# quarterwave0/LithographySimulator

Hardware: AMD Instinct MI355X
Metric: Abbe source-points x image-pixels per second (higher is better)
Workload: dtype f32

## Files before the change

lithographysimulator_amd/csrc/engine_kernels.hpp:

```cpp
#pragma once
#include <hip/hip_runtime.h>

#include "engine_common.hpp"
#include "abbe_plan.hpp"
#include "fft_core.hpp"
#include "wave_fft.hpp"

namespace litho {

template <int LOG2N>
struct Launch {
    using F = LineFFT<LOG2N, +1>;
    static constexpr int L = (F::T >= 64) ? 1 : 64 / F::T;
    static constexpr int THREADS = F::T * L;
#ifndef LITHO_NBUF
#define LITHO_NBUF 1
#endif
    static constexpr int NBUF = (LOG2N <= 12) ? LITHO_NBUF : 1;
    static constexpr size_t LDS_EXCH = (size_t)L * NBUF * F::LDS_LINE;
    static constexpr size_t LDS_BYTES = sizeof(float2) * (LDS_EXCH + F::LDS_TW);
#ifndef LITHO_WG_PER_CU
#define LITHO_WG_PER_CU 3
#endif
    static constexpr int WG_PER_CU = LOG2N <= 12 ? LITHO_WG_PER_CU : (LOG2N == 13 ? 2 : 1);
    static constexpr int WAVES = (THREADS / 256 > 0 ? THREADS / 256 : 1) * WG_PER_CU;
};


typedef unsigned int u32x2 __attribute__((ext_vector_type(2)));
static constexpr unsigned BUF_OOB = 0xFFFF0000u;

__device__ __forceinline__ __amdgpu_buffer_rsrc_t make_rsrc(const void* base, size_t bytes) {
    return __builtin_amdgcn_make_buffer_rsrc(const_cast<void*>(base), 0, (int)(unsigned)bytes, 0x00020000);
}
__device__ __forceinline__ float2 buf_load_c64(__amdgpu_buffer_rsrc_t r, unsigned off) {
    const u32x2 v = __builtin_amdgcn_raw_buffer_load_b64(r, off, 0, 0);
    return make_float2(__uint_as_float(v.x), __uint_as_float(v.y));
}
#ifndef LITHO_XSTORE_AUX
#define LITHO_XSTORE_AUX 16
#endif
template <int LOG2N> inline constexpr int t_store_aux = LOG2N >= 11 ? LITHO_XSTORE_AUX : 0;
typedef unsigned int u32x4 __attribute__((ext_vector_type(4)));
template <int AUX = 0>
__device__ __forceinline__ void buf_store_c64x2(__amdgpu_buffer_rsrc_t r, unsigned off, float2 a, float2 b) {
    u32x4 w;
    w.x = __float_as_uint(a.x); w.y = __float_as_uint(a.y);
    w.z = __float_as_uint(b.x); w.w = __float_as_uint(b.y);
    __builtin_amdgcn_raw_buffer_store_b128(w, r, off, 0, AUX);
}
template <int AUX = 0>
__device__ __forceinline__ void buf_store_c64(__amdgpu_buffer_rsrc_t r, unsigned off, float2 v) {
    u32x2 w;
    w.x = __float_as_uint(v.x);
    w.y = __float_as_uint(v.y);
    __builtin_amdgcn_raw_buffer_store_b64(w, r, off, 0, AUX);
}

__device__ __forceinline__ unsigned t_offset(const PassGeom& g, unsigned a, unsigned q) {
    return ((((q >> g.tcl) * g.rows + a) << g.tcl) + (q & ((1u << g.tcl) - 1u)));
}

typedef unsigned int uint2v __attribute__((ext_vector_type(2)));

__device__ __forceinline__ void touch_vgpr(float2& v) { asm volatile("" : "+v"(v.x), "+v"(v.y)); }
__device__ __forceinline__ void diag_keep(float2 v, unsigned o) { asm volatile("" ::"v"(v.x), "v"(v.y), "v"(o)); }

__device__ __forceinline__ const float* pack_weights() { return nullptr; }
__device__ __forceinline__ const float* pack_weights(const float* w) { return w; }

template <int LOG2N, int RL, bool PRUNED, int NP, int RP = 1, typename... Wt>
__global__ __launch_bounds__(Launch<LOG2N>::THREADS, (RP == 2 ? Launch<LOG2N>::WAVES / Launch<LOG2N>::WG_PER_CU * 2 : Launch<LOG2N>::WAVES)) void k_xpass_abbe(
    const float2* __restrict__ P, const float2* __restrict__ M, const int* __restrict__ shifts,
    float2* __restrict__ Tbuf, const float2* __restrict__ twtab, PassGeom g, int nb, int chunk, Wt... wts)
{
    constexpr bool WT = sizeof...(Wt) != 0;
    static_assert(sizeof...(Wt) <= 1 && !(WT && RP == 2), "weighted x-pass: one weight list, one row per workgroup (a weighted call ignores the row-pair knob)");
    [[maybe_unused]] const float* weights = pack_weights(wts...);
    using F = LineFFT<LOG2N, +1>;
    using LC = Launch<LOG2N>;
    constexpr unsigned IN = PRUNED ? natural_in_mask(RL) : 0xFFFFu;
    constexpr unsigned OUT = out_mask(RL);
    extern __shared__ __attribute__((aligned(16))) unsigned char smem_raw[];
    float2* smem = reinterpret_cast<float2*>(smem_raw);
    const int lt = threadIdx.x % F::T, lg = threadIdx.x / F::T;
    float2* lds = smem + (size_t)lg * LC::NBUF * F::LDS_LINE;

    typename F::Twiddles tw;
    F::load_twiddles(tw, twtab, lt, smem + LC::LDS_EXCH, threadIdx.x, LC::THREADS);

    static_assert(RP == 1 || (RP == 2 && NP == 1 && LC::L == 1), "row pairs: one plane, one line per workgroup");
    int a;
    if constexpr (LC::L == 1) {
        const int b = blockIdx.x, xcd = b & 7, i = b >> 3;
        a = ((i >> 2) * 32 + xcd * 4 + (i & 3)) * RP;
    } else {
        a = blockIdx.x * LC::L + lg;
    }
    const bool active = a < g.rows;
    const bool active1 = a + 1 < g.rows;
    const int r = g.ky0 + g.c + a;
    const size_t plane_bytes = (size_t)g.pn * g.pn * sizeof(float2);
    const __amdgpu_buffer_rsrc_t rM = make_rsrc(M, plane_bytes);

    unsigned koff[16];
    float2 pv[NP * RP][16];
    static_for<0, 16>([&](auto e_) {
        constexpr int e = decltype(e_)::value;
        if constexpr ((IN >> e) & 1u) {
            int k;
            const bool ok = centred_index(lt + F::T * e, F::N, g.kx0, g.kx1, k) && active;
            koff[e] = ok ? (unsigned)(g.c + k) : BUF_OOB;
        }
    });
    static_for<0, NP * RP>([&](auto p_) {
        constexpr int p = decltype(p_)::value;
        const __amdgpu_buffer_rsrc_t rP = make_rsrc(P + (size_t)(RP == 1 ? p : 0) * g.pn * g.pn, plane_bytes);
        static_for<0, 16>([&](auto e_) {
            constexpr int e = decltype(e_)::value;
            if constexpr ((IN >> e) & 1u)
                pv[p][e] = buf_load_c64(rP, koff[e] != BUF_OOB ? ((unsigned)(r + (RP == 1 ? 0 : p)) * g.pn + koff[e]) * 8u : BUF_OOB);
        });
    });
    unsigned toff[16];
    static_for<0, 16>([&](auto m_) {
        constexpr int m = decltype(m_)::value;
        if constexpr ((OUT >> m) & 1u) {
            int u;
            const bool ok = centred_index(lt + F::T * m, F::N, -g.c, g.pn - g.c, u) && active;
            const unsigned q = (unsigned)(u + g.c);
            toff[m] = ok ? t_offset(g, a, q) * 8u : BUF_OOB;
        }
    });

    const int s_begin = blockIdx.y * chunk;
    const int s_end = min(nb, s_begin + chunk);
    auto load_window = [&](int s, int rr, float2 (&mv)[16]) {
        const int dy = shifts[2 * s], dx = shifts[2 * s + 1];
        const unsigned mrow = (unsigned)(r + rr + dy) * g.pn + dx;
        static_for<0, 16>([&](auto e_) {
            constexpr int e = decltype(e_)::value;
            if constexpr ((IN >> e) & 1u)
#ifdef LITHO_DIAG_XNOLOAD
                mv[e] = make_float2((float)((mrow + koff[e]) & 1023u), 1.0f);
#else
                mv[e] = buf_load_c64(rM, koff[e] != BUF_OOB ? (mrow + koff[e]) * 8u : BUF_OOB);
#endif
        });
    };

    int flip = 0;
    float2 mnext[16];
    [[maybe_unused]] float wnext = 1.f;
    if (s_begin < s_end) load_window(s_begin, 0, mnext);
    if constexpr (WT) { if (s_begin < s_end) wnext = weights[s_begin]; }
    static_for<0, 16>([&](auto e_) {
        constexpr int e = decltype(e_)::value;
        if constexpr ((IN >> e) & 1u) touch_vgpr(mnext[e]);
    });
    const unsigned row1 = active1 ? (8u << g.tcl) : 0x80000000u;
    float2 held[RP == 2 ? 16 : 1];
    const bool hi8 = (threadIdx.x & 8) != 0;
    unsigned offc = 0, offd = 0;
    if constexpr (RP == 2) {
        const unsigned tileb = (unsigned)g.rows * (8u << g.tcl);
        offc = hi8 ? row1 - tileb : 0u;
        offd = hi8 ? 0u : row1 + tileb;
    }
    for (int s = s_begin; s < s_end; ++s) {
        static_for<0, RP>([&](auto rr_) {
            constexpr int rr = decltype(rr_)::value;
            float2 mv[16];
            static_for<0, 16>([&](auto e_) {
                constexpr int e = decltype(e_)::value;
                if constexpr ((IN >> e) & 1u) mv[e] = mnext[e];
            });
            [[maybe_unused]] float amp = 1.f;
            if constexpr (WT) amp = sqrtf(wnext);
#ifndef LITHO_XPASS_NO_PREFETCH
            if constexpr (rr + 1 < RP) load_window(s, rr + 1, mnext);
            else load_window(s + 1 < s_end ? s + 1 : s, 0, mnext);
#else
            if constexpr (rr + 1 < RP) load_window(s, rr + 1, mnext);
            else if (s + 1 < s_end) load_window(s + 1, 0, mnext);
#endif
            if constexpr (WT) {
                wnext = weights[s + 1 < s_end ? s + 1 : s];
                static_for<0, 16>([&](auto e_) {
                    constexpr int e = decltype(e_)::value;
                    if constexpr ((IN >> e) & 1u) mv[e] = make_float2(amp * mv[e].x, amp * mv[e].y);
                });
            }
            static_for<0, NP>([&](auto p_) {
                constexpr int p = decltype(p_)::value;
                float2 x[16];
                static_for<0, 16>([&](auto e_) {
                    constexpr int e = decltype(e_)::value;
                    if constexpr ((IN >> e) & 1u) x[e] = cmul(pv[RP == 1 ? p : rr][e], mv[e]);
                    else x[e] = make_float2(0.f, 0.f);
                });
                F::template run<LC::NBUF>(x, tw, lds, lt, flip);
                const __amdgpu_buffer_rsrc_t rT =
                    make_rsrc(Tbuf + ((size_t)p * nb + s) * g.t_point, (size_t)g.t_point * sizeof(float2));
                if constexpr (RP == 2 && rr == 0) {
                    static_for<0, 16>([&](auto m_) { held[decltype(m_)::value] = x[decltype(m_)::value]; });
                } else {
                    static_for<0, 16>([&](auto m_) {
                        constexpr int m = decltype(m_)::value;
#ifdef LITHO_DIAG_XNOSTORE
                        if constexpr ((OUT >> m) & 1u) diag_keep(x[m], toff[m]);
#elif defined(LITHO_DIAG_XSTORE_L2)
                        if constexpr ((OUT >> m) & 1u) buf_store_c64(rT, toff[m] == BUF_OOB ? BUF_OOB : (toff[m] & 0xFFFFFu), x[m]);
#else
                        if constexpr ((OUT >> m) & 1u) {
                            if constexpr (RP == 2) {
                                if (active) {
                                    const float bx = __uint_as_float(__builtin_amdgcn_update_dpp(0u, __float_as_uint(x[m].x), 0x128, 0xF, 0xF, false));
                                    const float by = __uint_as_float(__builtin_amdgcn_update_dpp(0u, __float_as_uint(x[m].y), 0x128, 0xF, 0xF, false));
                                    buf_store_c64<t_store_aux<LOG2N>>(rT, toff[m] + offc, hi8 ? make_float2(bx, by) : held[m]);
                                    buf_store_c64<t_store_aux<LOG2N>>(rT, toff[m] + offd, hi8 ? held[m] : make_float2(bx, by));
                                }
                            } else {
                                buf_store_c64<t_store_aux<LOG2N>>(rT, toff[m], x[m]);
                            }
                        }
#endif
                    });
                }
            });
        });
    }
}

template <int LOG2N, typename... Wt>
__global__ __launch_bounds__(Launch<LOG2N - 1>::THREADS, Launch<LOG2N - 1>::WAVES) void k_xpass_split(
    const float2* __restrict__ P, const float2* __restrict__ M, const int* __restrict__ shifts,
    float2* __restrict__ Tbuf, const float2* __restrict__ twtab, PassGeom g, int nb, int chunk, Wt... wts)
{
    constexpr bool WT = sizeof...(Wt) != 0;
    static_assert(sizeof...(Wt) <= 1, "one weight list");
    [[maybe_unused]] const float* weights = pack_weights(wts...);
    using F = LineFFT<LOG2N - 1, +1>;
    using LC = Launch<LOG2N - 1>;
    static_assert(LC::L == 1, "split x-pass: one row per workgroup");
    constexpr unsigned IN = natural_in_mask(0), OUT = out_mask(1);
    extern __shared__ __attribute__((aligned(16))) unsigned char smem_raw[];
    float2* smem = reinterpret_cast<float2*>(smem_raw);
    const int lt = threadIdx.x;
    float2* lds = smem;

    typename F::Twiddles tw;
// ... 680 lines not shown
```

lithographysimulator_amd/csrc/wave_kernels.hpp:

```cpp
#pragma once
#include "engine_kernels.hpp"

namespace litho {

template <int LOG2N>
struct WaveShape {
    static_assert(LOG2N >= 10 && LOG2N <= 12, "wave-per-line y-pass: N = 1024 .. 4096 (N = 8192: k_ypass_pair)");
    static constexpr int LS = LOG2N / 2;
    static constexpr int D = 1 << (LOG2N - 2 * LS);
    using W = WaveSq<LS>;
    static constexpr int S = W::S;
    static constexpr int THREADS = 256;
    static constexpr int UNITS = THREADS / S;
    static constexpr int COLS = UNITS / D;
    static constexpr int TILES = COLS / 4;
    static constexpr int JLIVE = S * D / 8;
    static constexpr size_t LDS_BYTES = (size_t)(THREADS / 64) * W::LDS_FLOATS * sizeof(float);
#ifndef LITHO_WAVE32_MINWAVES
#define LITHO_WAVE32_MINWAVES 4
#endif
    static constexpr int MINWAVES = LS == 5 ? LITHO_WAVE32_MINWAVES : 2;
};

template <int TC, int COLS>
__device__ __forceinline__ int wave_first_column(int b)
{
    constexpr int WPT = TC > COLS ? TC / COLS : 1;
    if constexpr (WPT == 1) return b * COLS;
    else return (((b / (8 * WPT)) * 8 + (b & 7)) * TC) + ((b >> 3) % WPT) * COLS;
}
template <int TC, int COLS>
static inline int wave_grid_x(int pn)
{
    constexpr int WPT = TC > COLS ? TC / COLS : 1;
    if constexpr (WPT == 1) return (pn + COLS - 1) / COLS;
    else return WPT * (((pn + TC - 1) / TC + 7) / 8 * 8);
}

typedef unsigned int u32x4v __attribute__((ext_vector_type(4)));
#ifndef LITHO_YLOAD_AUX
#define LITHO_YLOAD_AUX 0
#endif

template <int LOG2N, int TC, bool FULL = false>
__global__ __launch_bounds__(WaveShape<LOG2N>::THREADS, WaveShape<LOG2N>::MINWAVES) void k_ypass_wave(
    const float2* __restrict__ Tbuf, float* __restrict__ slab, const float2* __restrict__ twtab,
    PassGeom g, int nb, int G, int gstride)
{
    static_assert(TC == 4 || TC == 8, "T tiles are 4 or 8 columns wide");
    using WS = WaveShape<LOG2N>;
    using W = typename WS::W;
    static_assert(!FULL || WS::D == 1, "full-output variant: one unit per column");
    constexpr int S = WS::S, D = WS::D, JLIVE = FULL ? 2 * WS::JLIVE : WS::JLIVE, N = 1 << LOG2N;
    constexpr int NACC = FULL ? S : S / 2;
    auto kept_k2 = [](int i) constexpr { return FULL ? i : (i < S / 4 ? i : S / 2 + i); };
    extern __shared__ __attribute__((aligned(16))) unsigned char smem_raw[];
    float* smem = reinterpret_cast<float*>(smem_raw);
    const int lane = threadIdx.x & 63, wv = threadIdx.x >> 6;
    const int l = lane & (S - 1);
    const int unit = wv * W::LINES + (lane >> WS::LS);
    const int p = unit % D;
    const int colg = unit / D;
    float* lds = smem + wv * W::LDS_FLOATS;
    typename W::LaneTwiddles tw;
    float2* twlds = reinterpret_cast<float2*>(smem_raw + WS::LDS_BYTES);
    if constexpr (FULL) {
        W::fill_lane_twiddle_table(twlds, twtab, D, threadIdx.x, WS::THREADS);
        __syncthreads();
    } else {
        W::load_lane_twiddles(tw, twtab, l, D);
    }
    const float2 tl = twtab[l * p];

    const int qx = wave_first_column<TC, WS::COLS>(blockIdx.x) + colg;
    const int tile = __builtin_amdgcn_readfirstlane(qx / TC);
    const int col = qx & (TC - 1);
    const int plane = blockIdx.y / G, grp = blockIdx.y - plane * G;
    Tbuf += (size_t)plane * nb * g.t_point;
    slab += (size_t)plane * gstride * g.nt * 4 * g.pn;
    const bool active = tile * TC < g.pn;
    float acc[NACC];
    static_for<0, NACC>([&](auto i) { acc[i] = 0.f; });

    constexpr int RB = 8 * TC;
    const unsigned tile_bytes = active ? (unsigned)g.rows * RB : 0u;
    const unsigned vb = (unsigned)(l - g.ky0) * RB + (unsigned)col * 8u;
    auto slot_off = [&](int j) { return vb + (unsigned)(j <= JLIVE ? RB * S * j : RB * S * j - RB * S * S); };

    for (int s = grp; s < nb; s += G) {
#ifndef LITHO_WAVE_FULL_NOSYNC
        if constexpr (FULL) __builtin_amdgcn_s_barrier();
#endif
        const __amdgpu_buffer_rsrc_t rT =
            make_rsrc(Tbuf + (size_t)s * g.t_point + (size_t)(active ? tile : 0) * g.rows * TC, tile_bytes);
        float2 x[S];
#ifndef LITHO_WAVE_FULL_NOPAIR
        if constexpr (FULL && TC == 8) {
            float2* const mine = reinterpret_cast<float2*>(lds);
            float2* const theirs = reinterpret_cast<float2*>(smem + (wv ^ 1) * W::LDS_FLOATS);
            const unsigned vbp = vb - (unsigned)(col & 1) * 8u;
            auto pair_off = [&](int j) { return vbp + (unsigned)(j <= JLIVE ? RB * S * j : RB * S * j - RB * S * S); };
            static_for<JLIVE + 1, S - JLIVE>([&](auto j_) { x[decltype(j_)::value] = make_float2(0.f, 0.f); });
            const bool even_wave = (__builtin_amdgcn_readfirstlane(wv) & 1) == 0;
            if (even_wave) {
                static_for<0, JLIVE + 1>([&](auto j_) {
                    constexpr int j = decltype(j_)::value;
                    const u32x4v v = __builtin_amdgcn_raw_buffer_load_b128(rT, pair_off(j), 0, 0);
                    x[j] = make_float2(__uint_as_float(v.x), __uint_as_float(v.y));
                    theirs[j * 64 + lane] = make_float2(__uint_as_float(v.z), __uint_as_float(v.w));
                });
            } else {
                static_for<S - JLIVE, S>([&](auto j_) {
                    constexpr int j = decltype(j_)::value;
                    const u32x4v v = __builtin_amdgcn_raw_buffer_load_b128(rT, pair_off(j), 0, 0);
                    x[j] = make_float2(__uint_as_float(v.z), __uint_as_float(v.w));
                    theirs[(j - (S - JLIVE)) * 64 + lane] = make_float2(__uint_as_float(v.x), __uint_as_float(v.y));
                });
            }
            __syncthreads();
            if (even_wave) {
                static_for<S - JLIVE, S>([&](auto j_) { constexpr int j = decltype(j_)::value; x[j] = mine[(j - (S - JLIVE)) * 64 + lane]; });
            } else {
                static_for<0, JLIVE + 1>([&](auto j_) { constexpr int j = decltype(j_)::value; x[j] = mine[j * 64 + lane]; });
            }
            asm volatile("" ::: "memory");
        } else
#endif
        static_for<0, S>([&](auto j_) {
            constexpr int j = decltype(j_)::value;
            if constexpr (j <= JLIVE || j >= S - JLIVE) {
                float2 v = buf_load_c64(rT, slot_off(j));
                if constexpr (D > 1) {
                    if (p) {
                        constexpr int e = (S * j) % N;
                        constexpr double ang = 6.283185307179586476925 * e / N;
                        constexpr float sgn = (j >= S - JLIVE) ? -1.f : 1.f;
                        const float2 cj = make_float2(sgn * (float)__builtin_cos(ang), sgn * (float)__builtin_sin(ang));
                        v = cmul(cmul(v, cj), tl);
                    }
                }
                x[j] = v;
            } else {
                x[j] = make_float2(0.f, 0.f);
            }
        });
        if constexpr (FULL) W::template run_lds_tw<true>(x, twlds, lds, lane);
        else W::run(x, tw, lds, lane);
        static_for<0, NACC>([&](auto i_) {
            constexpr int i = decltype(i_)::value;
            constexpr int k2 = kept_k2(i);
            const float2 v = x[W::brev(k2)];
            acc[i] = fmaf(v.x, v.x, fmaf(v.y, v.y, acc[i]));
        });
    }

    if (!active || qx >= g.pn) return;
    float* srow = slab + ((size_t)grp * g.nt * 4 + qx) * g.pn;
    static_for<0, NACC>([&](auto i_) {
        constexpr int i = decltype(i_)::value;
        constexpr int k2 = kept_k2(i);
        const int n = l + S * k2;
        const int v = n < S * S / 2 ? n : n - S * S;
        srow[D * v + p + g.c] += acc[i];
    });
}

template <int NW>
struct CoopShape {
    static_assert(NW == 4, "four waves share four columns (32 bytes) of a tile row");
    static constexpr int S = 64, N = 4096, JLIVE = 16, NLIVE = 2 * JLIVE + 1;
    static constexpr int STAGE_FLOATS = NLIVE * 64 * 2 + 16;
    static constexpr int WAVE_FLOATS = STAGE_FLOATS >= WaveSq<6>::LDS_FLOATS ? STAGE_FLOATS : WaveSq<6>::LDS_FLOATS + 16;
    static_assert(WAVE_FLOATS >= WaveSq<6>::LDS_FLOATS, "the staging area holds the transpose matrix");
    static constexpr size_t LDS_BYTES = NW * (size_t)WAVE_FLOATS * sizeof(float) + (size_t)WaveSq<6>::TW_LDS_FLOAT2 * sizeof(float2);
    static constexpr int PARTS = 16 / NW;
    static inline int grid_x(int pn) { return PARTS * (((pn + 15) / 16 + 7) / 8 * 8); }
};

#ifdef LITHO_DIAG_COOP_NOLOAD
#define COOP_LOAD(r, off) u32x4v{(off), 0x3f800000u, (off) >> 3, 0x3f000000u}
#else
#define COOP_LOAD(r, off) __builtin_amdgcn_raw_buffer_load_b128(r, off, 0, 0)
#endif
template <int LOG2N, int NW>
__global__ __launch_bounds__(64 * NW, 2) void k_ypass_coop(
    const float2* __restrict__ Tbuf, float* __restrict__ slab, const float2* __restrict__ twtab,
    PassGeom g, int nb, int G, int gstride)
{
    static_assert(LOG2N == 12, "cooperative-loading y-pass over 16-column tiles: N = 4096");
    using W = WaveSq<6>;
    using CS = CoopShape<NW>;
    constexpr int S = CS::S, N = CS::N, JLIVE = CS::JLIVE, NLIVE = CS::NLIVE, TC = 16, RB = 8 * TC;
    constexpr int PART_BYTES = 8 * NW;
    extern __shared__ __attribute__((aligned(16))) unsigned char smem_raw[];
    float* smem = reinterpret_cast<float*>(smem_raw);
// ... 225 lines not shown
            prefetch(snext);
        }
        W::dft_dif(x);
#endif
        static_for<0, S>([&](auto i_) {
            constexpr int i = decltype(i_)::value;
            const float2 v = x[W::brev(i)];
            acc[i] = fmaf(v.x, v.x, fmaf(v.y, v.y, acc[i]));
        });
    }
    if (!active || qx >= g.pn) return;
    float* srow = slab + ((size_t)grp * g.nt * 4 + qx) * g.pn;
    static_for<0, S>([&](auto i_) {
        constexpr int i = decltype(i_)::value;
        const int n = lane + S * i;
        const int v = n < S * S / 2 ? n : n - S * S;
        srow[v + g.c] += acc[i];
    });
}

template <int LOG2N, int TC>
__global__ __launch_bounds__(256, 2) void k_ypass_pair(
    const float2* __restrict__ Tbuf, float* __restrict__ slab, const float2* __restrict__ twtab,
    PassGeom g, int nb, int G, int gstride)
{
    static_assert(LOG2N == 13, "pair-of-waves y-pass: N = 8192");
    using W = WaveSq<6>;
    constexpr int S = 64, N = 1 << LOG2N;
    extern __shared__ __attribute__((aligned(16))) unsigned char smem_raw[];
    float* smem = reinterpret_cast<float*>(smem_raw);
    const int lane = threadIdx.x & 63;
    const int wv = __builtin_amdgcn_readfirstlane(threadIdx.x >> 6);
    const int par = wv & 1, pair = wv >> 1;
    float* mat_own = smem + wv * W::LDS_FLOATS;
    const float* mat_other = smem + (wv ^ 1) * W::LDS_FLOATS;
    typename W::LaneTwiddles tw;
    W::load_lane_twiddles(tw, twtab, lane + S * par, 1);

    static_assert(TC == 4 || TC == 8, "T tiles are 4 or 8 columns wide");
    const int qx = wave_first_column<TC, 2>(blockIdx.x) + pair;
    const int tile = qx / TC, col = qx & (TC - 1);
    const int plane = blockIdx.y / G, grp = blockIdx.y - plane * G;
    Tbuf += (size_t)plane * nb * g.t_point;
    slab += (size_t)plane * gstride * g.nt * 4 * g.pn;
    const bool active = tile * TC < g.pn;
    float acc[S / 2];
    static_for<0, S / 2>([&](auto i) { acc[i] = 0.f; });

    constexpr int RB = 8 * TC;
    const unsigned tile_bytes = active ? (unsigned)g.rows * RB : 0u;
    const unsigned vb = (unsigned)(lane + S * par - g.ky0) * RB + (unsigned)col * 8u;
    auto slot_off = [&](int j) { return vb + (unsigned)(j <= 8 ? RB * 2 * S * j : RB * 2 * S * j - RB * N); };

    for (int s = grp; s < nb; s += G) {
        const __amdgpu_buffer_rsrc_t rT =
            make_rsrc(Tbuf + (size_t)s * g.t_point + (size_t)(active ? tile : 0) * g.rows * TC, tile_bytes);
        float2 x[S];
        static_for<0, S>([&](auto j_) {
            constexpr int j = decltype(j_)::value;
            if constexpr (j <= 8 || j >= S - 8) x[j] = buf_load_c64(rT, slot_off(j));
            else x[j] = make_float2(0.f, 0.f);
        });
        W::run_pair(x, tw, mat_own, mat_other, lane, par);
        static_for<0, S / 2>([&](auto i_) {
            constexpr int i = decltype(i_)::value;
            constexpr int k2 = i < S / 4 ? i : S / 2 + i;
            const float2 v = x[W::brev(k2)];
            acc[i] = fmaf(v.x, v.x, fmaf(v.y, v.y, acc[i]));
        });
    }

    if (!active || qx >= g.pn) return;
    float* srow = slab + ((size_t)grp * g.nt * 4 + qx) * g.pn;
    static_for<0, S / 2>([&](auto i_) {
        constexpr int i = decltype(i_)::value;
        constexpr int k2 = i < S / 4 ? i : S / 2 + i;
        constexpr int ubase = k2 < S / 2 ? 2 * S * k2 : 2 * S * k2 - N;
        srow[ubase + lane + S * par + g.c] += acc[i];
    });
}

template <int LOG2N, int TC, bool FULL = false, int GW = 1>
__global__ __launch_bounds__(256 * GW, 2) void k_ypass_rect(
    const float2* __restrict__ Tbuf, float* __restrict__ slab, const float2* __restrict__ twtab,
    PassGeom g, int nb, int G, int gstride)
{
    static_assert(GW == 1 || GW == 2, "one or two groups per workgroup");
    static_assert(LOG2N >= 8 && LOG2N <= 11, "multi-column-per-wave y-pass: N = 256 (full output only), 512, 1024, 2048");
    static_assert(TC == 2 || TC == 4 || TC == 8, "T tiles are 2, 4 or 8 columns wide");
    static_assert(LOG2N >= 9 || FULL, "N = 256: the coarse-grid transform of 256^2 images");
    using W = WaveSq<6>;
    constexpr int S = 64, N = 1 << LOG2N, NL = (S * S) / N, H = S / NL;
    constexpr int JL = FULL ? H / 4 : H / 8;
    constexpr int NACC = FULL ? S : S / 2;
    auto kept_k2 = [](int i) constexpr { return FULL ? i : (i < S / 4 ? i : S / 2 + i); };
    static_assert(NL <= TC || NL == 2 * TC, "the wave's columns sit in one T tile, or in two adjacent ones (N = 256)");
    constexpr int NT = NL <= TC ? 1 : 2;
    constexpr int QT = NL / 2 / NT;
    extern __shared__ __attribute__((aligned(16))) unsigned char smem_raw[];
    float* smem = reinterpret_cast<float*>(smem_raw);
    const int lane = threadIdx.x & 63;
    const int wv = __builtin_amdgcn_readfirstlane(threadIdx.x >> 6);
    const int cw = wv & 3, gl = wv >> 2;
    float* lds = smem + wv * W::LDS_FLOATS;
    typename W::LaneTwiddles tw;
    W::load_lane_twiddles(tw, twtab, lane, 1);

    const int qx0 = wave_first_column<TC, 4 * NL>(blockIdx.x) + NL * cw;
    const int tile = qx0 / TC, col = qx0 & (TC - 1);
    const int GB = G / GW;
    const int plane = blockIdx.y / GB, gb = blockIdx.y - plane * GB;
    const int grp = gb * GW + gl;
    Tbuf += (size_t)plane * nb * g.t_point;
    slab += (size_t)plane * gstride * g.nt * 4 * g.pn;
    const bool active = tile * TC < g.pn;
    float acc[NACC];
    static_for<0, NACC>([&](auto i) { acc[i] = 0.f; });

    constexpr int RB = 8 * TC;
    const unsigned tile_bytes = active ? (unsigned)g.rows * RB : 0u;
    const unsigned vb = (unsigned)(lane - g.ky0) * RB + (unsigned)col * 8u;
    auto slot_off = [&](int j) { return vb + (unsigned)(j <= JL ? RB * S * j : RB * S * j - RB * N); };

    for (int s = grp; s < nb; s += G) {
        __amdgpu_buffer_rsrc_t rTs[NT];
        static_for<0, NT>([&](auto t_) {
            constexpr int t = decltype(t_)::value;
            rTs[t] = make_rsrc(Tbuf + (size_t)s * g.t_point + (size_t)(active ? tile + t : 0) * g.rows * TC, tile_bytes);
        });
        float2 x[S];
        static_for<0, H>([&](auto j_) {
            constexpr int j = decltype(j_)::value;
            static_for<0, NL / 2>([&](auto q_) {
                constexpr int q = decltype(q_)::value;
                if constexpr (j <= JL || j >= H - JL) {
                    const u32x4v v = __builtin_amdgcn_raw_buffer_load_b128(rTs[q / QT], slot_off(j) + 16u * (q % QT), 0, LITHO_YLOAD_AUX);
                    x[(2 * q) * H + j] = make_float2(__uint_as_float(v.x), __uint_as_float(v.y));
                    x[(2 * q + 1) * H + j] = make_float2(__uint_as_float(v.z), __uint_as_float(v.w));
                } else {
                    x[(2 * q) * H + j] = make_float2(0.f, 0.f);
                    x[(2 * q + 1) * H + j] = make_float2(0.f, 0.f);
                }
            });
        });
        W::template run_rect<NL>(x, tw, lds, lane);
        static_for<0, NACC>([&](auto i_) {
            constexpr int i = decltype(i_)::value;
            constexpr int k2 = kept_k2(i);
            const float2 v = x[W::brev(k2)];
            acc[i] = fmaf(v.x, v.x, fmaf(v.y, v.y, acc[i]));
        });
    }

    if constexpr (GW == 2) {
        if (gl == 1) static_for<0, NACC>([&](auto i_) { constexpr int i = decltype(i_)::value; lds[i * 64 + lane] = acc[i]; });
        __syncthreads();
        if (gl == 1) return;
        const float* other = smem + (wv + 4) * W::LDS_FLOATS;
        static_for<0, NACC>([&](auto i_) { constexpr int i = decltype(i_)::value; acc[i] += other[i * 64 + lane]; });
    }
    const int qx = qx0 + lane / H, m = lane & (H - 1);
    if (!active || qx >= g.pn) return;
    float* srow = slab + ((size_t)gb * g.nt * 4 + qx) * g.pn;
    static_for<0, NACC>([&](auto i_) {
        constexpr int i = decltype(i_)::value;
        constexpr int k2 = kept_k2(i);
        constexpr int ubase = k2 < S / 2 ? H * k2 : H * k2 - N;
#if defined(LITHO_DIAG_YFLUSH_STORE)
        srow[ubase + m + g.c] = acc[i];
#elif defined(LITHO_DIAG_YFLUSH_NONE)
        if (acc[i] == 12345.678f) srow[ubase + m + g.c] = acc[i];
#else
        srow[ubase + m + g.c] += acc[i];
#endif
    });
}


template <int LOG2N, bool FULL = false, typename... Wt>
__global__ __launch_bounds__(256, 2) void k_xpass_rect(
    const float2* __restrict__ P, const float2* __restrict__ M, const int* __restrict__ shifts,
    float2* __restrict__ Tbuf, const float2* __restrict__ twtab, PassGeom g, int nb, int chunk, Wt... wts)
{
    constexpr bool WT = sizeof...(Wt) != 0;
    static_assert(sizeof...(Wt) <= 1, "one weight list");
    [[maybe_unused]] const float* weights = pack_weights(wts...);
    static_assert(LOG2N >= 9 && LOG2N <= 11, "multi-row-per-wave x-pass: N = 512, 1024, 2048");
    using W = WaveSq<6>;
    constexpr int S = 64, N = 1 << LOG2N, NL = (S * S) / N, H = S / NL, JL = FULL ? H / 4 : H / 8, TC = 8;
    constexpr int NOUT = FULL ? S : S / 2;
    extern __shared__ __attribute__((aligned(16))) unsigned char smem_raw[];
    float* smem = reinterpret_cast<float*>(smem_raw);
    const int lane = threadIdx.x & 63;
    const int wv = __builtin_amdgcn_readfirstlane(threadIdx.x >> 6);
    float* lds = smem + wv * W::LDS_FLOATS;
    typename W::LaneTwiddles tw;
    W::load_lane_twiddles(tw, twtab, lane, 1);

    const int a0 = (blockIdx.x * 4 + wv) * NL;
    const int s_begin = blockIdx.y * chunk;
    const int s_end = min(nb, s_begin + chunk);
    if (a0 >= g.rows) return;

    const unsigned win_bytes = (unsigned)(g.kx1 - g.kx0) * 8u;
    const unsigned vb = (unsigned)(lane - g.kx0) * 8u;
    auto slot_off = [&](int j) { return vb + (unsigned)(j <= JL ? 512 * j : 512 * j - 8 * N); };
    const int r0 = g.ky0 + g.c + a0;

    const int oline = lane / H, om = lane & (H - 1);
    const bool ovalid = a0 + oline < g.rows;
    const unsigned rowstride = (unsigned)g.rows * (TC * 8u);
    const unsigned obase = ovalid ? (unsigned)(om >> 3) * rowstride + (unsigned)(a0 + oline) * (TC * 8u) + (unsigned)(om & 7) * 8u
                                  : BUF_OOB;

    for (int s = s_begin; s < s_end; ++s) {
        const int dy = shifts[2 * s], dx = shifts[2 * s + 1];
        [[maybe_unused]] float amp = 1.f;
        if constexpr (WT) amp = sqrtf(weights[s]);
        float2 x[S];
        static_for<0, NL>([&](auto q_) {
            constexpr int line = decltype(q_)::value;
            const bool rvalid = a0 + line < g.rows;
            const __amdgpu_buffer_rsrc_t rP =
                make_rsrc(P + (size_t)(r0 + (rvalid ? line : 0)) * g.pn + g.c + g.kx0, rvalid ? win_bytes : 0u);
            const __amdgpu_buffer_rsrc_t rM =
                make_rsrc(M + (size_t)(r0 + (rvalid ? line : 0) + dy) * g.pn + dx + g.c + g.kx0, rvalid ? win_bytes : 0u);
            static_for<0, H>([&](auto j_) {
                constexpr int j = decltype(j_)::value;
                if constexpr (j <= JL || j >= H - JL) {
                    if constexpr (WT) {
                        const float2 m = buf_load_c64(rM, slot_off(j));
                        x[line * H + j] = cmul(buf_load_c64(rP, slot_off(j)), make_float2(amp * m.x, amp * m.y));
                    } else {
                        x[line * H + j] = cmul(buf_load_c64(rP, slot_off(j)), buf_load_c64(rM, slot_off(j)));
                    }
                }
                else x[line * H + j] = make_float2(0.f, 0.f);
            });
        });
        W::template run_rect<NL>(x, tw, lds, lane);
        const __amdgpu_buffer_rsrc_t rT =
            make_rsrc(Tbuf + (size_t)s * g.t_point, (size_t)g.t_point * sizeof(float2));
        static_for<0, NOUT>([&](auto i_) {
            constexpr int i = decltype(i_)::value;
            constexpr int k2 = FULL ? i : (i < S / 4 ? i : S / 2 + i);
            constexpr int ub = k2 < S / 2 ? H * k2 : H * k2 - N;
            const unsigned tile_off = (unsigned)((ub + g.c) >> 3) * rowstride;
            buf_store_c64(rT, obase == BUF_OOB ? BUF_OOB : obase + tile_off, x[W::brev(k2)]);
        });
    }
}

template <int LOG2N>
hipError_t launch_xpass_rect(const float2* P, const float2* M, const int* shifts, const float* wts, float2* T, const float2* tw,
                             const PassGeom& g, int nb, int chunk, hipStream_t st)
{
    if constexpr (LOG2N >= 9 && LOG2N <= 11) {
        if (g.tcl != 3) return hipErrorNotSupported;
        static LdsOnce once;
        constexpr size_t lds = 4 * WaveSq<6>::LDS_FLOATS * sizeof(float);
        constexpr int NL = 4096 >> LOG2N;
        const int groups = (g.rows + NL - 1) / NL;
        const dim3 grid((groups + 3) / 4, (nb + chunk - 1) / chunk);
        if (wts) {
            if (g.N == g.pn) {
                static LdsOnce once_full_wt;
                auto kern = k_xpass_rect<LOG2N, true, const float*>;
                hipError_t e = set_lds(once_full_wt, kern, lds);
                if (e != hipSuccess) return e;
                hipLaunchKernelGGL(kern, grid, dim3(256), lds, st, P, M, shifts, T, tw, g, nb, chunk, wts);
                note_kernel(0, "k_xpass_rect<%d, true, float const*>", LOG2N);
                return hipGetLastError();
            }
            static LdsOnce once_wt;
            auto kern = k_xpass_rect<LOG2N, false, const float*>;
            hipError_t e = set_lds(once_wt, kern, lds);
            if (e != hipSuccess) return e;
            hipLaunchKernelGGL(kern, grid, dim3(256), lds, st, P, M, shifts, T, tw, g, nb, chunk, wts);
            note_kernel(0, "k_xpass_rect<%d, false, float const*>", LOG2N);
            return hipGetLastError();
        }
        if (g.N == g.pn) {
            static LdsOnce once_full;
            auto kern = k_xpass_rect<LOG2N, true>;
            hipError_t e = set_lds(once_full, kern, lds);
            if (e != hipSuccess) return e;
            hipLaunchKernelGGL(kern, grid, dim3(256), lds, st, P, M, shifts, T, tw, g, nb, chunk);
            note_kernel(0, "k_xpass_rect<%d, true>", LOG2N);
            return hipGetLastError();
        }
        auto kern = k_xpass_rect<LOG2N>;
        hipError_t e = set_lds(once, kern, lds);
        if (e != hipSuccess) return e;
        hipLaunchKernelGGL(kern, grid, dim3(256), lds, st, P, M, shifts, T, tw, g, nb, chunk);
        note_kernel(0, "k_xpass_rect<%d, false>", LOG2N);
        return hipGetLastError();
    } else {
        return hipErrorNotSupported;
    }
}

template <int LOG2N, int TC>
static hipError_t launch_ypass_wave_tc(const float2* T, float* slab, const float2* tw, const PassGeom& g, int nb, int planes, int G,
                     int gstride, hipStream_t st)
{
    constexpr size_t lds4 = 4 * WaveSq<6>::LDS_FLOATS * sizeof(float);
    if (g.N == g.pn) {
        if constexpr (LOG2N == 12) {
            static LdsOnce once;
            constexpr size_t ldsf = lds4 + (size_t)WaveSq<6>::TW_LDS_FLOAT2 * sizeof(float2);
            auto kern = k_ypass_wave<LOG2N, TC, true>;
            hipError_t e = set_lds(once, kern, ldsf);
// ... 138 lines not shown
```

Baseline: 497.7 billion.

## Split y-pass accumulator flush across both wave groups and early-exit idle x-pass blocks

In the y-pass for N of 2048 and above, the final cross-group reduction is rebuilt so both wave groups each sum and flush half of the accumulator bins, instead of one group sitting idle while the other does all the read-modify-write. Each group loads the old slab values before the barrier so that latency overlaps the LDS exchange, and stores through buffer stores with a cache-policy aux field. In the x-pass, workgroups whose row index is out of range now return before loading twiddles, avoiding wasted loads. The split path adds register pressure for the prefetched old values and depends on the aux bits chosen.

```diff
diff --git a/lithographysimulator_amd/csrc/engine_kernels.hpp b/lithographysimulator_amd/csrc/engine_kernels.hpp
--- a/lithographysimulator_amd/csrc/engine_kernels.hpp
+++ b/lithographysimulator_amd/csrc/engine_kernels.hpp
@@ -86,17 +86,17 @@
     const int lt = threadIdx.x % F::T, lg = threadIdx.x / F::T;
     float2* lds = smem + (size_t)lg * LC::NBUF * F::LDS_LINE;
 
-    typename F::Twiddles tw;
-    F::load_twiddles(tw, twtab, lt, smem + LC::LDS_EXCH, threadIdx.x, LC::THREADS);
-
     static_assert(RP == 1 || (RP == 2 && NP == 1 && LC::L == 1), "row pairs: one plane, one line per workgroup");
     int a;
     if constexpr (LC::L == 1) {
         const int b = blockIdx.x, xcd = b & 7, i = b >> 3;
         a = ((i >> 2) * 32 + xcd * 4 + (i & 3)) * RP;
+        if (a >= g.rows) return;
     } else {
         a = blockIdx.x * LC::L + lg;
     }
+    typename F::Twiddles tw;
+    F::load_twiddles(tw, twtab, lt, smem + LC::LDS_EXCH, threadIdx.x, LC::THREADS);
     const bool active = a < g.rows;
     const bool active1 = a + 1 < g.rows;
     const int r = g.ky0 + g.c + a;
diff --git a/lithographysimulator_amd/csrc/wave_kernels.hpp b/lithographysimulator_amd/csrc/wave_kernels.hpp
--- a/lithographysimulator_amd/csrc/wave_kernels.hpp
+++ b/lithographysimulator_amd/csrc/wave_kernels.hpp
@@ -41,6 +41,10 @@
 #ifndef LITHO_YLOAD_AUX
 #define LITHO_YLOAD_AUX 0
 #endif
+#ifndef LITHO_YFLUSH_AUX
+#define LITHO_YFLUSH_AUX 17
+#endif
+template <int LOG2N> inline constexpr bool y_flush_split = LOG2N >= 11;
 
 template <int LOG2N, int TC, bool FULL = false>
 __global__ __launch_bounds__(WaveShape<LOG2N>::THREADS, WaveShape<LOG2N>::MINWAVES) void k_ypass_wave(
@@ -572,12 +576,50 @@
         });
     }
 
-    if constexpr (GW == 2) {
+    if constexpr (GW == 2 && !y_flush_split<LOG2N>) {
         if (gl == 1) static_for<0, NACC>([&](auto i_) { constexpr int i = decltype(i_)::value; lds[i * 64 + lane] = acc[i]; });
         __syncthreads();
         if (gl == 1) return;
         const float* other = smem + (wv + 4) * W::LDS_FLOATS;
         static_for<0, NACC>([&](auto i_) { constexpr int i = decltype(i_)::value; acc[i] += other[i * 64 + lane]; });
+    }
+    if constexpr (GW == 2 && y_flush_split<LOG2N>) {
+        constexpr int HB = NACC / 2;
+        const int qx = qx0 + lane / H, m = lane & (H - 1);
+        float* srow = slab + ((size_t)gb * g.nt * 4 + qx) * g.pn;
+        const bool live = active && qx < g.pn;
+        auto bin_of = [&](int i) constexpr { const int k2 = kept_k2(i); return k2 < S / 2 ? H * k2 : H * k2 - N; };
+        float old[HB];
+        const float* other = smem + (wv ^ 4) * W::LDS_FLOATS;
+        auto fetch = [&](auto h_) {
+            constexpr int h = decltype(h_)::value;
+#if !defined(LITHO_DIAG_YFLUSH_STORE) && !defined(LITHO_DIAG_YFLUSH_NONE)
+            if (live) static_for<0, HB>([&](auto i_) { constexpr int i = decltype(i_)::value; old[i] = srow[bin_of(h * HB + i) + m + g.c]; });
+#endif
+            static_for<0, HB>([&](auto i_) { constexpr int i = decltype(i_)::value; lds[i * 64 + lane] = acc[(1 - h) * HB + i]; });
+        };
+        auto flush = [&](auto h_) {
+            constexpr int h = decltype(h_)::value;
+            [[maybe_unused]] const __amdgpu_buffer_rsrc_t rS =
+                make_rsrc(slab + (size_t)gb * g.nt * 4 * g.pn, (size_t)g.nt * 4 * g.pn * sizeof(float));
+            static_for<0, HB>([&](auto i_) {
+                constexpr int i = decltype(i_)::value;
+                const float o = other[i * 64 + lane];
+                const float sum = h == 0 ? acc[i] + o : o + acc[HB + i];
+#if defined(LITHO_DIAG_YFLUSH_STORE)
+                srow[bin_of(h * HB + i) + m + g.c] = sum;
+#elif defined(LITHO_DIAG_YFLUSH_NONE)
+                if (sum == 12345.678f) srow[bin_of(h * HB + i) + m + g.c] = sum;
+#else
+                __builtin_amdgcn_raw_buffer_store_b32(__float_as_uint(old[i] + sum), rS, (unsigned)(qx * g.pn + bin_of(h * HB + i) + m + g.c) * 4u, 0, LITHO_YFLUSH_AUX);
+#endif
+            });
+        };
+        if (gl == 0) fetch(std::integral_constant<int, 0>{}); else fetch(std::integral_constant<int, 1>{});
+        lds_barrier();
+        if (!live) return;
+        if (gl == 0) flush(std::integral_constant<int, 0>{}); else flush(std::integral_constant<int, 1>{});
+        return;
     }
     const int qx = qx0 + lane / H, m = lane & (H - 1);
     if (!active || qx >= g.pn) return;
```

After: 501.9 billion (median of 6 runs). Within noise of the previous version (+0.8%).
